# EdwardFerdian/4DFlowNet

Measured on AMD Instinct MI355X. Metric: 3D patches/sec (train step, patch=24, res×2), higher is better.
Workload: dtype f32; 1 GPU; cfg2 train_step: patch_size=24 res_increase=2 batch=8/GPU low_resblock=8 hi_resblock=4 fp32; global_batch=8, parallelism=dp1, collective=none

## Files before the change

4dflownet_amd/_lib.py:

```python
import contextlib
import ctypes
import os

from . import build as _build

_HERE = os.path.dirname(os.path.abspath(__file__))
LIB_PATH = os.path.join(_HERE, "lib4dflow_hip.so")
TEST_LIB_PATH = os.path.join(_HERE, "lib4dflow_hip_test.so")

c_fp = ctypes.c_void_p
c_i = ctypes.c_int
c_i64 = ctypes.c_int64
c_u64 = ctypes.c_uint64
c_f = ctypes.c_float
c_sz = ctypes.c_size_t

SIGNATURES = {
    "fdn_version": (c_i, []),
    "fdn_last_error": (ctypes.c_char_p, []),
    "fdn_input_features": (c_i, [c_fp] * 8 + [c_i64, c_fp]),
    "fdn_pack_conv64_weights": (c_i, [c_fp, c_fp, c_fp, c_fp]),
    "fdn_conv3d_fwd": (c_i, [c_fp] * 7 + [c_i] * 10 + [c_f, c_i, c_fp]),
    "fdn_conv3d_dgrad": (c_i, [c_fp] * 4 + [c_i] * 10 + [c_fp]),
    "fdn_conv_cout1_dgrad_folded": (c_i, [c_fp, c_fp, c_fp, c_i, c_f, c_fp, c_fp, c_fp, c_sz, c_i, c_i, c_i, c_i, c_i, c_i, c_fp]),
    "fdn_conv_cout1_dgrad_folded_mask": (c_i, [c_fp, c_fp, c_fp, c_i, c_f, c_fp, c_fp, c_fp, c_sz, c_i, c_i, c_i, c_i, c_i, c_i, c_fp]),
    "fdn_fold_halo": (c_i, [c_fp, c_fp, c_fp, c_i, c_fp, c_fp, c_i, c_f, c_fp, c_i, c_i, c_i, c_i, c_i, c_fp]),
    "fdn_conv3d_dgrad_fused": (c_i, [c_fp] * 5 + [c_i, c_f, c_fp, c_i, c_i, c_i, c_i, c_i, c_fp]),
    "fdn_conv64_mask_ok": (c_i, [c_i] * 5),
    "fdn_conv64_fwd_mask": (c_i, [c_fp] * 6 + [c_i] * 5 + [c_f, c_i, c_fp]),
    "fdn_conv64_dgrad_fused_mask": (c_i, [c_fp] * 5 + [c_i, c_f, c_fp, c_i, c_i, c_i, c_i, c_i, c_fp]),
    "fdn_conv64_dgrad_fused_multi": (c_i, [c_fp, c_fp, c_i] + [c_fp] * 4 + [c_i, c_f, c_fp, c_i, c_i, c_i, c_i, c_i, c_fp]),
    "fdn_conv3d_dgrad_fused_part": (c_i, [c_fp] * 5 + [c_i, c_f, c_fp, c_i, c_i, c_i, c_i, c_i, c_i, c_fp]),
    "fdn_fold_halo_border": (c_i, [c_fp, c_fp, c_fp, c_i, c_fp, c_fp, c_i, c_f, c_fp, c_i, c_i, c_i, c_i, c_fp]),
    "fdn_conv1x1_dgrad": (c_i, [c_fp] * 6 + [c_i64, c_fp]),
    "fdn_conv3d_wgrad_workspace_bytes": (c_sz, [c_i] * 7),
    "fdn_conv3d_wgrad_batch_workspace_bytes": (c_sz, [c_i] * 5),
    "fdn_conv3d_wgrad_batch": (c_i, [c_fp, c_fp, c_fp, c_fp, c_i, c_fp, c_sz] + [c_i] * 5 + [c_fp]),
    "fdn_conv3d_wgrad": (c_i, [c_fp] * 6 + [c_sz] + [c_i] * 10 + [c_fp]),
    "fdn_upsample_trilinear_fwd": (c_i, [c_fp, c_fp] + [c_i] * 6 + [c_fp]),
    "fdn_upsample_trilinear_bwd": (c_i, [c_fp, c_fp, c_i, c_f, c_fp] + [c_i] * 6 + [c_fp]),
    "fdn_loss_metrics": (c_i, [c_fp] * 8 + [c_i, c_i64, c_fp]),
    "fdn_loss_metrics_div": (c_i, [c_fp] * 5 + [c_f] + [c_fp] * 3 + [c_i] * 4 + [c_fp]),
    "fdn_loss_metrics_act": (c_i, [c_fp] * 5 + [c_f, c_f, c_i] + [c_fp] * 3 + [c_i] * 4 + [c_fp]),
    "fdn_loss_metrics_kind": (c_i, [c_fp] * 5 + [c_i, c_f, c_f, c_f, c_i] + [c_fp] * 3 + [c_i] * 4 + [c_fp]),
    "fdn_volume_metrics": (c_i, [c_fp, c_i, c_fp, c_fp, c_i, c_fp, c_fp] + [c_i] * 4 + [c_fp]),
    "fdn_gather_patches": (c_i, [c_fp, c_fp, c_i, c_i, c_fp]),
    "fdn_input_features_volume": (c_i, [c_fp] + [c_i] * 8 + [c_i64, c_i, c_fp, c_fp, c_fp]),
    "fdn_stitch_patches": (c_i, [c_fp, c_fp] + [c_i] * 9 + [c_i64, c_i, c_fp]),
    "fdn_stitch_patches_finish": (c_i, [c_fp, c_fp, c_fp] + [c_i] * 9 + [c_i64, c_i, c_fp]),
    "fdn_pack_patch_cores": (c_i, [c_fp, c_fp, c_i, c_i, c_i, c_fp]),
    "fdn_input_features_volume_oriented": (c_i, [c_fp] + [c_i] * 8 + [c_i64, c_i, c_i, c_i, c_fp, c_fp, c_fp]),
    "fdn_unrotate_accumulate": (c_i, [c_fp, c_fp] + [c_i] * 6 + [c_fp]),
    "fdn_input_features_volume_strided": (c_i, [c_fp] + [c_i] * 8 + [c_i64, c_i, c_i, c_i, c_i, c_fp, c_fp, c_fp]),
    "fdn_blend_patches": (c_i, [c_fp, c_fp] + [c_i] * 10 + [c_i64, c_i, c_fp]),
    "fdn_finish_volume": (c_i, [c_fp, c_fp, c_fp] + [c_i] * 4 + [c_fp]),
    "fdn_kspace_downsample_workspace_bytes": (c_sz, [c_i] * 7),
    "fdn_kspace_downsample": (c_i, [c_fp, c_fp, c_fp] + [c_i] * 7 + [c_fp, c_u64, c_u64] + [c_fp] * 5),
    "fdn_l2_sumsq": (c_i, [c_fp, c_fp, c_i64, c_fp, c_fp]),
    "fdn_adam_step": (c_i, [c_fp] * 5 + [c_i64] + [c_f] * 5 + [c_fp, c_fp, c_fp]),
    "fdn_adam_step_dev": (c_i, [c_fp] * 5 + [c_i64, c_fp] + [c_f] * 4 + [c_fp, c_fp, c_fp]),
    "fdn_adam_step_masked": (c_i, [c_fp] * 6 + [c_i64, c_f, c_fp] + [c_f] * 4 + [c_fp, c_fp, c_fp]),
    "fdn_sum_partials": (c_i, [c_fp, c_i, c_fp, c_fp]),
    "fdn_grad_accumulate": (c_i, [c_fp, c_fp, c_i64, c_i, c_fp]),
    "fdn_l2_sumsq_partials": (c_i, [c_fp, c_fp, c_i64, c_fp, c_fp]),
    "fdn_grad_sumsq_partials": (c_i, [c_fp] * 4 + [c_i64, c_f, c_fp, c_fp, c_fp]),
    "fdn_clip_scale": (c_i, [c_fp, c_i, c_f, c_fp, c_fp]),
    "fdn_adam_step_clipped": (c_i, [c_fp] * 6 + [c_i64, c_f, c_fp] + [c_f] * 4 + [c_fp, c_fp, c_f, c_fp, c_fp]),
    "fdn_adam_step_ema": (c_i, [c_fp] * 6 + [c_i64, c_f, c_fp] + [c_f] * 4 + [c_fp, c_fp, c_f, c_fp, c_f, c_i, c_fp, c_fp]),
    "fdn_pack_conv64_weights_batch": (c_i, [c_fp, c_fp, c_i, c_fp, c_fp]),
    "fdn_conv64_pack_streams": (c_i, [c_i] * 6),
    "fdn_pack_conv64_weights_batch_streams": (c_i, [c_fp, c_fp, c_i, c_fp, c_i, c_i, c_fp]),
    "fdn_pack_conv64_weights_bf16": (c_i, [c_fp, c_fp, c_fp, c_fp]),
    "fdn_pack_conv64_weights_bf16_batch": (c_i, [c_fp, c_fp, c_i, c_fp, c_fp]),
# ... 118 lines not shown
```

4dflownet_amd/csrc/elementwise.hip:

```cpp
#include "fdn_common.h"

namespace {

__device__ __forceinline__ float norm3(float a, float b, float c) {
    return sqrtf(__builtin_fmaf(c, c, __builtin_fmaf(a, a, b * b)));
}

template <typename T>
__global__ void input_features_kernel(const float* __restrict__ u, const float* __restrict__ v, const float* __restrict__ w,
                                      const float* __restrict__ mu, const float* __restrict__ mv,
                                      const float* __restrict__ mw, T* __restrict__ phase, T* __restrict__ pc, int64_t nvox) {
    for (int64_t i = (int64_t)blockIdx.x * blockDim.x + threadIdx.x; i < nvox; i += (int64_t)gridDim.x * blockDim.x) {
        const float a = u[i], b = v[i], c = w[i];
        const float ma = mu[i], mb = mv[i], mc = mw[i];
        const float speed = norm3(a, b, c);
        const float mag = norm3(ma, mb, mc);
        fdn_st1(phase + i * 3 + 0, a); fdn_st1(phase + i * 3 + 1, b); fdn_st1(phase + i * 3 + 2, c);
        fdn_st1(pc + i * 3 + 0, mag * speed); fdn_st1(pc + i * 3 + 1, mag); fdn_st1(pc + i * 3 + 2, speed);
    }
}

struct InputGeom {
    int32_t P, X, Y, Z;
    int32_t nx, ny, nz, orient;
// ... 571 lines not shown
            const float wgt = MSE ? 2.f * c0 : c0;
            const float gu = pen_psi<KIND>(du, kp, kp2) * wgt, gv = pen_psi<KIND>(dv, kp, kp2) * wgt, gw = pen_psi<KIND>(dw, kp, kp2) * wgt;
            if (out_act == FDN_ACT_TANH) tanh_grad_store(pred, g * 3, dpred + g * 3, gu, gv, gw);
            else { dpred[g * 3] = gu; dpred[g * 3 + 1] = gv; dpred[g * 3 + 2] = gw; }
        }
    }
    const float a = block_sum(sf, red);
    const float b = block_sum(snf, red);
    const float c = block_sum(srel, red);
    if (threadIdx.x == 0) {
        float* part = scratch + (size_t)gridDim.y * 8 + ((size_t)n * gridDim.x + blockIdx.x) * nparts;
        part[0] = a; part[1] = b; part[2] = c;
        if (nparts == 5) { part[3] = 0.f; part[4] = 0.f; }
    }
}

__global__ __launch_bounds__(256) __attribute__((amdgpu_waves_per_eu(7))) void loss_main_kernel(const float* __restrict__ pred, const float* __restrict__ uh,
                                                         const float* __restrict__ vh, const float* __restrict__ wh,
                                                         const float* __restrict__ mask, float* __restrict__ scratch,
                                                         float* __restrict__ dpred, int64_t V, int D, int H, int W, float div_w,
                                                         int nparts, float nf_w, int out_act, int kind, float kp) {
    __shared__ float red[4];
    if (kind == FDN_LOSS_MSE) {
        loss_body<FDN_LOSS_MSE>(pred, uh, vh, wh, mask, scratch, dpred, V, D, H, W, div_w, nparts, nf_w, out_act, 0.f, red);
        return;
    }
    int other = kind;
    asm volatile("" : "+s"(other));
    if (other == FDN_LOSS_MAE) loss_body<FDN_LOSS_MAE>(pred, uh, vh, wh, mask, scratch, dpred, V, D, H, W, div_w, nparts, nf_w, out_act, 0.f, red);
    else if (other == FDN_LOSS_HUBER) loss_body<FDN_LOSS_HUBER>(pred, uh, vh, wh, mask, scratch, dpred, V, D, H, W, div_w, nparts, nf_w, out_act, kp, red);
    else loss_body<FDN_LOSS_CHARBONNIER>(pred, uh, vh, wh, mask, scratch, dpred, V, D, H, W, div_w, nparts, nf_w, out_act, kp, red);
}

__global__ __launch_bounds__(64) void loss_finalize_kernel(const float* __restrict__ scratch, float* __restrict__ out, int N, int nblk,
                                                           int nparts, float div_w, float nf_w) {
    const int n = blockIdx.x;
    const float* part = scratch + (size_t)N * 8 + (size_t)n * nblk * nparts;
    float sf = 0.f, sn = 0.f, sr = 0.f, sdf = 0.f, sdn = 0.f;
    if (nparts == 5) {
        for (int b = threadIdx.x; b < nblk; b += 64) {
            sf += part[b * 5]; sn += part[b * 5 + 1]; sr += part[b * 5 + 2]; sdf += part[b * 5 + 3]; sdn += part[b * 5 + 4];
        }
        for (int o = 32; o > 0; o >>= 1) { sdf += __shfl_down(sdf, o, 64); sdn += __shfl_down(sdn, o, 64); }
    } else {
        for (int b = threadIdx.x; b < nblk; b += 64) { sf += part[b * 3]; sn += part[b * 3 + 1]; sr += part[b * 3 + 2]; }
    }
    for (int o = 32; o > 0; o >>= 1) { sf += __shfl_down(sf, o, 64); sn += __shfl_down(sn, o, 64); sr += __shfl_down(sr, o, 64); }
    if (threadIdx.x) return;
    const float sm = scratch[n * 8 + 0], snf = scratch[n * 8 + 1];
    const int nc = nparts == 5 ? 5 : 4;
    out[n * nc + 0] = sf / (sm + 1.f) + nf_w * (sn / (snf + 1.f));
    out[n * nc + 1] = sr / (sm + 1.f) * 100.f;
    out[n * nc + 2] = sm;
    out[n * nc + 3] = snf;
    if (nparts == 5) out[n * 5 + 4] = div_w * (sdf / (sm + 1.f) + nf_w * (sdn / (snf + 1.f)));
}

__global__ __launch_bounds__(1024) void l2_sumsq_kernel(const float* __restrict__ w, const uint8_t* __restrict__ isk,
                                                         int64_t n, float* __restrict__ out) {
    __shared__ float red[16];
    float s0 = 0.f, s1 = 0.f, s2 = 0.f, s3 = 0.f;
    int64_t i = threadIdx.x;
    for (; i + 3 * 1024 < n; i += 4 * 1024) {
        const float a0 = isk[i] ? w[i] : 0.f, a1 = isk[i + 1024] ? w[i + 1024] : 0.f;
        const float a2 = isk[i + 2048] ? w[i + 2048] : 0.f, a3 = isk[i + 3072] ? w[i + 3072] : 0.f;
        s0 += a0 * a0; s1 += a1 * a1; s2 += a2 * a2; s3 += a3 * a3;
    }
    for (; i < n; i += 1024)
// ... 267 lines not shown
    FDN_REQUIRE(hb == 1 || hb == 2, "fdn_upsample_trilinear_bwd: %d rows per block", hb);
    if (int rc = hb == 2 ? launch(std::integral_constant<int, 2>{}) : launch(std::integral_constant<int, 1>{})) return rc;
    FDN_CHECK_LAUNCH("upsample_bwd_kernel");
    return FDN_OK;
}
extern "C" int fdn_upsample_trilinear_fwd(const float* x, float* y, int N, int D, int H, int W, int C, int R, void* stream) {
    return upsample_fwd_t<float>(x, y, N, D, H, W, C, R, stream);
}
extern "C" int fdn_upsample_trilinear_bwd(const float* dy, const float* y_prev, int act, float alpha, float* dx, int N, int D,
                                          int H, int W, int C, int R, void* stream) {
    return upsample_bwd_t<float>(dy, y_prev, act, alpha, dx, N, D, H, W, C, R, stream);
}
extern "C" int fdn_upsample_trilinear_fwd_bf16(const uint16_t* x, uint16_t* y, int N, int D, int H, int W, int C, int R,
                                               void* stream) {
    return upsample_fwd_t<uint16_t>(x, y, N, D, H, W, C, R, stream);
}
extern "C" int fdn_upsample_trilinear_bwd_bf16(const uint16_t* dy, const uint16_t* y_prev, int act, float alpha, uint16_t* dx,
                                               int N, int D, int H, int W, int C, int R, void* stream) {
    return upsample_bwd_t<uint16_t>(dy, y_prev, act, alpha, dx, N, D, H, W, C, R, stream);
}

static int loss_launch(const char* who, const float* pred, const float* uh, const float* vh, const float* wh, const float* mask, float* out,
                       float* dpred, float* scratch, int N, int64_t V, int D, int H, int W, float div_w, int nparts, void* stream,
                       float nf_w = 1.f, int out_act = FDN_ACT_NONE, int kind = FDN_LOSS_MSE, float kind_param = 0.f) {
    hipStream_t s = (hipStream_t)stream;
    hipError_t e = hipMemsetAsync(scratch, 0, (size_t)N * 8 * sizeof(float), s);
    if (e != hipSuccess) { fdn_set_error("%s: memset: %s", who, hipGetErrorString(e)); return FDN_ERR_HIP; }
    const int gx = grid_for(V, FDN_LOSS_BLOCKS);
    hipLaunchKernelGGL(mask_sums_kernel, dim3(gx < 16 ? gx : 16, N), dim3(256), 0, s, mask, scratch, V);
    FDN_CHECK_LAUNCH("mask_sums_kernel");
    hipLaunchKernelGGL(loss_main_kernel, dim3(gx, N), dim3(256), 0, s, pred, uh, vh, wh, mask, scratch, dpred, V, D, H, W, div_w, nparts,
                       nf_w, out_act, kind, kind_param);
    FDN_CHECK_LAUNCH("loss_main_kernel");
    hipLaunchKernelGGL(loss_finalize_kernel, dim3(N), dim3(64), 0, s, (const float*)scratch, out, N, gx, nparts, div_w, nf_w);
    FDN_CHECK_LAUNCH("loss_finalize_kernel");
    return FDN_OK;
}

extern "C" int fdn_loss_metrics(const float* pred, const float* uh, const float* vh, const float* wh, const float* mask,
                                float* out, float* dpred, float* scratch, int N, int64_t V, void* stream) {
    FDN_REQUIRE(pred && uh && vh && wh && mask && out && scratch && N > 0 && V > 0, "fdn_loss_metrics: bad argument");
    return loss_launch("fdn_loss_metrics", pred, uh, vh, wh, mask, out, dpred, scratch, N, V, 1, 1, 1, 0.f, 3, stream);
}

extern "C" int fdn_loss_metrics_div(const float* pred, const float* uh, const float* vh, const float* wh, const float* mask,
                                    float div_weight, float* out, float* dpred, float* scratch, int N, int D, int H, int W,
                                    void* stream) {
    FDN_REQUIRE(pred && uh && vh && wh && mask && out && scratch, "fdn_loss_metrics_div: NULL operand");
    FDN_REQUIRE(N > 0 && D > 0 && H > 0 && W > 0, "fdn_loss_metrics_div: extents N=%d D=%d H=%d W=%d must be positive", N, D, H, W);
    FDN_REQUIRE((int64_t)D * H * W <= (int64_t)INT32_MAX, "fdn_loss_metrics_div: %d x %d x %d voxels per sample exceed 2^31 - 1", D, H, W);
    FDN_REQUIRE(__builtin_isfinite(div_weight) && div_weight >= 0.f, "fdn_loss_metrics_div: div_weight %g must be finite and >= 0",
                (double)div_weight);
    return loss_launch("fdn_loss_metrics_div", pred, uh, vh, wh, mask, out, dpred, scratch, N, (int64_t)D * H * W, D, H, W, div_weight, 5,
                       stream);
}

extern "C" int fdn_loss_metrics_act(const float* pred, const float* uh, const float* vh, const float* wh, const float* mask,
                                    float div_weight, float non_fluid_weight, int out_act, float* out, float* dpred, float* scratch,
                                    int N, int D, int H, int W, void* stream) {
    FDN_REQUIRE(pred && uh && vh && wh && mask && out && scratch, "fdn_loss_metrics_act: NULL operand");
    FDN_REQUIRE(N > 0 && D > 0 && H > 0 && W > 0, "fdn_loss_metrics_act: extents N=%d D=%d H=%d W=%d must be positive", N, D, H, W);
    FDN_REQUIRE((int64_t)D * H * W <= (int64_t)INT32_MAX, "fdn_loss_metrics_act: %d x %d x %d voxels per sample exceed 2^31 - 1", D, H, W);
    FDN_REQUIRE(__builtin_isfinite(div_weight) && div_weight >= 0.f, "fdn_loss_metrics_act: div_weight %g must be finite and >= 0",
                (double)div_weight);
    FDN_REQUIRE(__builtin_isfinite(non_fluid_weight) && non_fluid_weight >= 0.f,
                "fdn_loss_metrics_act: non_fluid_weight %g must be finite and >= 0", (double)non_fluid_weight);
    if (out_act != FDN_ACT_NONE && out_act != FDN_ACT_TANH) {
// ... 215 lines not shown
```

4dflownet_amd/csrc/heads_mfma.hip:

```cpp
#include "fdn_common.h"
#include <type_traits>
#include <stdlib.h>

namespace {

__device__ __forceinline__ int clampi(int v, int hi) { return min(max(v, 0), hi); }

__device__ __forceinline__ float head_tanh(float z) {
    const float a = fabsf(z);
    const float s = a * a;
    float p = __fadd_rn(__fmul_rn(-5.70498872745e-3f, s), 2.06390887954e-2f);
    p = fmaf(p, s, -5.37397155531e-2f);
    p = fmaf(p, s, 1.33314422036e-1f);
    p = fmaf(p, s, -3.33332819422e-1f);
    const float q = 0.25f * a;
    const float e = __builtin_amdgcn_exp2f(11.54156033f * (q > 4.f ? 4.f : q));
    const float t = a < 0.625f ? fmaf(p * s, a, a) : 1.f - 2.f / (e + 1.f);
    return copysignf(t, z);
}
__device__ __forceinline__ float head_act(float z, int act, float alpha) {
    if (act == FDN_ACT_TANH) return head_tanh(z);
    return fdn_act(z, act, alpha);
}

// ... 144 lines not shown
}

}

template <typename T>
int fdn_head_fwd_launch(const T* x, const float* w, const float* bias, float* y, int N, int D, int H, int W, int ldy, int y_coff,
                        int act, float alpha, hipStream_t s, int xcd_walk) {
    const int ntd = (D + H_TD - 1) / H_TD, nth = (H + H_TH - 1) / H_TH, ntw = (W + H_TW - 1) / H_TW;
    const size_t lds = (size_t)27 * H_HVP * sizeof(float);
    if (int rc = fdn_func_max_lds((const void*)head_fwd_kernel<T>, (int)lds, "head_fwd")) return rc;
    const int ntiles = N * ntd * nth * ntw;
    const int iters = 3 * ((ntiles + 3 * 512 - 1) / (3 * 512));
    const int grid = (ntiles + iters - 1) / iters;
    FDN_PLAN("fam=head_fwd op=fwd dt=%s N=%d D=%d H=%d W=%d iters=%d last=%d grid=%d tiles=%d cus=%d", sizeof(T) == 2 ? "bf16" : "f32", N, D, H, W,
             iters, ntiles - (grid - 1) * iters, grid, ntiles, fdn_plan_cus());
    hipLaunchKernelGGL(head_fwd_kernel<T>, dim3((unsigned)grid), dim3(256), lds, s, x, w, bias, y, N, D, H, W, ntd, nth, ntw, iters,
                       ldy, y_coff, act, alpha, xcd_walk);
    FDN_CHECK_LAUNCH("head_fwd_kernel");
    return FDN_OK;
}
template int fdn_head_fwd_launch<float>(const float*, const float*, const float*, float*, int, int, int, int, int, int, int, float, hipStream_t, int);
template int fdn_head_fwd_launch<uint16_t>(const uint16_t*, const float*, const float*, float*, int, int, int, int, int, int, int, float, hipStream_t, int);

namespace {

template <typename T>
__global__ __launch_bounds__(256, 2) void head_dgrad_kernel(const float* __restrict__ dz, const float* __restrict__ w,
                                                            const T* __restrict__ yprev, int act, float alpha,
                                                            T* __restrict__ out, float* __restrict__ bpart, int N, int D, int H,
                                                            int W, int ntd, int nth, int ntw, int lddz, int dz_coff,
                                                            const uint16_t* __restrict__ ymask) {
    __shared__ float zs[2][H_HV + 8];
    __shared__ float bred[4][64];
    const int tid = threadIdx.x, lane = tid & 63, wave = tid >> 6;
    const int li = lane & 31, kh = lane >> 5;
    const int tiles_per_n = ntd * nth * ntw, ntiles = N * tiles_per_n;
    const float slope = act == FDN_ACT_RELU ? 0.f : (act == FDN_ACT_LEAKY ? alpha : 1.f);

    constexpr bool VROW = sizeof(T) == 4;
    typedef __bf16 bf16x8 __attribute__((ext_vector_type(8)));
    float wa[VROW ? 2 : 1][VROW ? 14 : 1];
    bf16x8 wbh[VROW ? 1 : 2][VROW ? 1 : 2], wbl[VROW ? 1 : 2][VROW ? 1 : 2];
#pragma unroll
    for (int m = 0; m < 2; ++m) {
        const int ch = VROW ? 32 * m + li : 32 * m + 16 * ((li >> 2) & 1) + (li & 3) + 4 * (li >> 3);
        if constexpr (VROW) {
#pragma unroll
            for (int s = 0; s < 14; ++s) wa[m][s] = (2 * s + kh) < 27 ? w[(2 * s + kh) * 64 + ch] : 0.f;
        } else {
#pragma unroll
            for (int blk = 0; blk < 2; ++blk)
#pragma unroll
                for (int j = 0; j < 8; ++j) {
                    const int t = 16 * blk + 8 * kh + j;
                    const float wv = t < 27 ? w[t * 64 + ch] : 0.f;
                    const __bf16 h = (__bf16)wv;
                    wbh[m][blk][j] = h;
                    wbl[m][blk][j] = (__bf16)(wv - (float)h);
                }
        }
    }
    struct TileOrg { int n, d, h, w; };
    auto decode = [&](int tile) {
        int b = min(tile, ntiles - 1);
        TileOrg o;
        o.n = b / tiles_per_n;
// ... 13 lines not shown
            float v = 0.f;
            if ((unsigned)qd < (unsigned)D && (unsigned)qh < (unsigned)H && (unsigned)qw < (unsigned)W)
                v = dz[((size_t)o.n * D * H * W + ((size_t)qd * H + qh) * W + qw) * lddz + dz_coff];
            dst[i] = v;
        }
    };
    float bsum[2][16];
#pragma unroll
    for (int m = 0; m < 2; ++m)
#pragma unroll
        for (int r = 0; r < 16; ++r) bsum[m][r] = 0.f;

    constexpr int NST = (H_HV + 255) / 256;
    float stv[NST];
    auto stage_load = [&](const TileOrg& o) {
#pragma unroll
        for (int u = 0; u < NST; ++u) {
            const int i = tid + 256 * u;
            const int zd = i / (H_XH * H_XW);
            const int r2 = i - zd * (H_XH * H_XW);
            const int zh = r2 / H_XW;
            const int qd = o.d + zd - 1, qh = o.h + zh - 1, qw = o.w + (r2 - zh * H_XW) - 1;
            float v = 0.f;
            if (i < H_HV && (unsigned)qd < (unsigned)D && (unsigned)qh < (unsigned)H && (unsigned)qw < (unsigned)W)
                v = dz[((size_t)o.n * D * H * W + ((size_t)qd * H + qh) * W + qw) * lddz + dz_coff];
            stv[u] = v;
        }
    };
    auto stage_store = [&](float* dst) {
#pragma unroll
        for (int u = 0; u < NST; ++u)
            if (tid + 256 * u < H_HV) dst[tid + 256 * u] = stv[u];
    };
    stage(decode(blockIdx.x), zs[0]);
    int par = 0;
    for (int tile = blockIdx.x; tile < ntiles; tile += gridDim.x, par ^= 1) {
        __syncthreads();
        const bool has_next = tile + (int)gridDim.x < ntiles;
        if (has_next) stage_load(decode(tile + gridDim.x));
        const TileOrg o = decode(tile);
        const float* z = zs[par];
#pragma unroll 1
        for (int mt = wave * 2; mt < wave * 2 + 2; ++mt) {
            const int vd = mt >> 1, vh = 4 * (mt & 1) + (li >> 3), vw = li & 7;
            const int gd = o.d + vd, gh = o.h + vh, gw = o.w + vw;
            float ym[2][16];
            fdn_u32x2 ymw[VROW ? 2 : 1][VROW ? 4 : 1];
            if constexpr (VROW) {
                if (ymask) {
                    const int pw = min(o.w + 4 * kh, W - 4), ph0 = o.h + 4 * (mt & 1);
                    const size_t nv = (size_t)N * D * H * W;
                    const size_t plane = (size_t)o.n * D * H * W + (size_t)min(gd, D - 1) * H * W;
#pragma unroll
                    for (int m = 0; m < 2; ++m)
#pragma unroll
                        for (int rr = 0; rr < 4; ++rr)
                            ymw[m][rr] = *(const fdn_u32x2*)(ymask + (size_t)(2 * m + (li >> 4)) * nv + plane + (size_t)min(ph0 + rr, H - 1) * W + pw);
                } else
                if (yprev) {
                    const int pw = o.w + 4 * kh, ph0 = o.h + 4 * (mt & 1);
                    const size_t plane = (size_t)o.n * D * H * W + (size_t)min(gd, D - 1) * H * W;
#pragma unroll
                    for (int r = 0; r < 16; ++r) {
                        const size_t e = (plane + (size_t)min(ph0 + (r >> 2), H - 1) * W + min(pw + (r & 3), W - 1)) * 64 + li;
                        ym[0][r] = fdn_ld1(yprev + e);
                        ym[1][r] = fdn_ld1(yprev + e + 32);
                    }
                }
            }
            constexpr int EVP = FdnVec<T>::E;
            float yq[VROW ? 1 : 2][VROW ? 1 : 16];
            unsigned ymk[2] = {0u, 0u};
            if constexpr (!VROW) {
                if (ymask) {
                    const size_t voxp = (size_t)o.n * D * H * W + ((size_t)min(gd, D - 1) * H + min(gh, H - 1)) * W + min(gw, W - 1);
                    ymk[0] = ymask[voxp * 4 + kh];
                    ymk[1] = ymask[voxp * 4 + 2 + kh];
                } else if (yprev) {
                    const size_t voxp = (size_t)o.n * D * H * W + ((size_t)min(gd, D - 1) * H + min(gh, H - 1)) * W + min(gw, W - 1);
#pragma unroll
                    for (int m = 0; m < 2; ++m)
#pragma unroll
                        for (int r0 = 0; r0 < 16; r0 += EVP) {
                            float t[EVP];
                            FdnVec<T>::ld(yprev + voxp * 64 + 32 * m + 16 * kh + r0, t);
#pragma unroll
                            for (int q = 0; q < EVP; ++q) yq[m][r0 + q] = t[q];
                        }
                }
            }
            float nb[3][3][3];
#pragma unroll
// ... 44 lines not shown
                for (int s = 0; s < 14; ++s) {
                    const int t0 = 2 * s, t1 = 2 * s + 1;
                    const float e0 = nb[t0 / 9][(t0 / 3) % 3][t0 % 3];
                    const float e1 = t1 < 27 ? nb[t1 / 9][(t1 / 3) % 3][t1 % 3] : 0.f;
                    const float bv = kh ? e1 : e0;
                    acc[0] = __builtin_amdgcn_mfma_f32_32x32x2f32(bv, wa[0][s], acc[0], 0, 0, 0);
                    acc[1] = __builtin_amdgcn_mfma_f32_32x32x2f32(bv, wa[1][s], acc[1], 0, 0, 0);
                }
            } else {
#pragma unroll
                for (int blk = 0; blk < 2; ++blk) {
                    bf16x8 ah, al;
#pragma unroll
                    for (int j = 0; j < 8; ++j) {
                        const int t0 = 16 * blk + j, t1 = 16 * blk + 8 + j;
                        const float e0 = nb[t0 / 9][(t0 / 3) % 3][t0 % 3];
                        const float e1 = t1 < 27 ? nb[(t1 % 27) / 9][((t1 % 27) / 3) % 3][t1 % 3] : 0.f;
                        const float av = kh ? e1 : e0;
                        const __bf16 h = (__bf16)av;
                        ah[j] = h;
                        al[j] = (__bf16)(av - (float)h);
                    }
#pragma unroll
                    for (int m = 0; m < 2; ++m) {
                        acc[m] = __builtin_amdgcn_mfma_f32_32x32x16_bf16(wbh[m][blk], ah, acc[m], 0, 0, 0);
                        acc[m] = __builtin_amdgcn_mfma_f32_32x32x16_bf16(wbh[m][blk], al, acc[m], 0, 0, 0);
                        acc[m] = __builtin_amdgcn_mfma_f32_32x32x16_bf16(wbl[m][blk], ah, acc[m], 0, 0, 0);
                    }
                }
            }
            if constexpr (VROW) {
                const int pw = o.w + 4 * kh, ph0 = o.h + 4 * (mt & 1);
                const size_t plane = (size_t)o.n * D * H * W + (size_t)min(gd, D - 1) * H * W;
#pragma unroll
                for (int r = 0; r < 16; ++r) {
                    const int qh = ph0 + (r >> 2), qw = pw + (r & 3);
                    const bool in2 = gd < D && qh < H && qw < W;
                    const size_t e = (plane + (size_t)min(qh, H - 1) * W + min(qw, W - 1)) * 64 + li;
#pragma unroll
                    for (int m = 0; m < 2; ++m) {
                        float v = acc[m][r];
                        if (ymask) v *= ((ymw[m][r >> 2][(r & 3) >> 1] >> (16 * (r & 1) + (li & 15))) & 1u) ? 1.f : slope;
                        else if (yprev) v *= ym[m][r] > 0.f ? 1.f : slope;
                        if (in2) {
                            fdn_st1(out + e + 32 * m, v);
                            bsum[m][0] += v;
                        }
                    }
                }
                continue;
            }
            const bool inside = gd < D && gh < H && gw < W;
            const size_t vox = (size_t)o.n * D * H * W + ((size_t)min(gd, D - 1) * H + min(gh, H - 1)) * W + min(gw, W - 1);
#pragma unroll
            for (int m = 0; m < 2; ++m) {
                const size_t e = vox * 64 + 32 * m + 16 * kh;
                constexpr int EV = FdnVec<T>::E;
#pragma unroll
                for (int r0 = 0; r0 < 16; r0 += EV) {
                    float v[EV];
#pragma unroll
                    for (int q = 0; q < EV; ++q) v[q] = acc[m][r0 + q];
                    if (!VROW && ymask) {
#pragma unroll
                        for (int q = 0; q < EV; ++q) v[q] *= ((ymk[m] >> (r0 + q)) & 1u) ? 1.f : slope;
                    } else if (yprev) {
#pragma unroll
                        for (int q = 0; q < EV; ++q) v[q] *= yq[VROW ? 0 : m][VROW ? 0 : r0 + q] > 0.f ? 1.f : slope;
                    }
                    if (inside) {
                        FdnVec<T>::st(out + e + r0, v);
#pragma unroll
                        for (int q = 0; q < EV; ++q) bsum[m][r0 + q] += v[q];
                    }
                }
            }
        }
        if (has_next) stage_store(zs[par ^ 1]);
    }
    if (bpart && VROW) {
#pragma unroll
        for (int m = 0; m < 2; ++m) {
            float v = bsum[m][0];
            v += __shfl_xor(v, 32, 64);
            if (kh == 0) bred[wave][32 * m + li] = v;
        }
        __syncthreads();
        if (tid < 64) bpart[(size_t)blockIdx.x * 64 + tid] = (bred[0][tid] + bred[1][tid]) + (bred[2][tid] + bred[3][tid]);
    } else if (bpart) {
#pragma unroll
        for (int m = 0; m < 2; ++m)
#pragma unroll
            for (int r = 0; r < 16; ++r) {
                float v = bsum[m][r];
                v += __shfl_xor(v, 1, 64); v += __shfl_xor(v, 2, 64); v += __shfl_xor(v, 4, 64);
                v += __shfl_xor(v, 8, 64); v += __shfl_xor(v, 16, 64);
                if (li == 0) bred[wave][32 * m + 16 * kh + r] = v;
            }
        __syncthreads();
        if (tid < 64) bpart[(size_t)blockIdx.x * 64 + tid] = (bred[0][tid] + bred[1][tid]) + (bred[2][tid] + bred[3][tid]);
    }
}

}

int fdn_head_dgrad_blocks(int N, int D, int H, int W) {
    const long long ntiles = (long long)N * ((D + H_TD - 1) / H_TD) * ((H + H_TH - 1) / H_TH) * ((W + H_TW - 1) / H_TW);
    return (int)(ntiles < 1024 ? ntiles : 1024);
}

template <typename T>
// ... 330 lines not shown
```

4dflownet_amd/ops.py:

```python
import ctypes
import functools
import math
import numbers
import operator
import struct

import numpy as np
import torch

from . import _lib
from ._lib import FdnError, check

ACT_NONE, ACT_RELU, ACT_LEAKY = 0, 1, 2
ACT_TANH = 3
ALGO_AUTO, ALGO_DIRECT, ALGO_WINO_W, ALGO_WINO_H2, ALGO_WINO_BF16X3 = 0, 1, 2, 3, 4
LEAKY_ALPHA = 0.2
CONV64_PACK_FLOATS = 423 * 64 * 64
ACT_DTYPE = torch.float32
PACK_ELEMS = CONV64_PACK_FLOATS


def _ptr(dtype, t, name="tensor", allow_none=False):
    if t is None:
        if allow_none:
# ... 708 lines not shown
        raise FdnError("grad_sumsq_partials: partials needs %d floats" % ADAM_PARTIALS)
    n = g.numel()
    for name, t in (("w", w), ("is_kernel", is_kernel), ("frozen", frozen)):
        if t is not None and t.numel() != n:
            raise FdnError("grad_sumsq_partials: %s holds %d elements for %d gradients" % (name, t.numel(), n))
    if l2_scale_dev is not None and (not l2_scale_dev.is_cuda or l2_scale_dev.dtype != torch.float32 or l2_scale_dev.numel() < 1):
        raise FdnError("grad_sumsq_partials: l2_scale_dev must hold one float32 on the GPU")
    check(_lib.load().fdn_grad_sumsq_partials(_p(g, "g"), _p(w, "w"), _pu8(is_kernel, "is_kernel"), _pu8(frozen, "frozen", allow_none=True), n,
                                              float(l2_grad_scale), _p(l2_scale_dev, "l2_scale_dev", allow_none=True), _p(partials, "partials"),
                                              _stream()), "fdn_grad_sumsq_partials")
    return partials


def clip_scale(partials, clip_norm, out=None):
    c32 = ctypes.c_float(float(clip_norm)).value
    if not (c32 > 0.0 and c32 != float("inf")):
        raise FdnError("clip_scale: clip_norm must be finite and > 0 in float32, got %r" % (clip_norm,))
    clip_norm = c32
    if out is None:
        out = torch.empty((2,), device=partials.device, dtype=torch.float32)
    elif out.numel() < 2:
        raise FdnError("clip_scale: out needs 2 floats")
    check(_lib.load().fdn_clip_scale(_p(partials, "partials"), partials.numel(), clip_norm, _p(out, "out"), _stream()), "fdn_clip_scale")
    return out


def sum_partials(partials, out=None):
    if out is None:
        out = torch.empty((1,), device=partials.device, dtype=torch.float32)
    check(_lib.load().fdn_sum_partials(_p(partials), partials.numel(), _p(out), _stream()), "fdn_sum_partials")
    return out


def pack_conv64_weights_batch(w_flat, w_offsets, packs, streams=None):
    n = w_offsets.numel()
    if w_offsets.dtype != torch.int64 or not w_offsets.is_cuda or packs.numel() != n * 2 * CONV64_PACK_FLOATS:
        raise FdnError("pack_conv64_weights_batch: bad offsets / packs")
    sf, sd = (PACK_STREAM_ALL, PACK_STREAM_ALL) if streams is None else streams
    check(_lib.load().fdn_pack_conv64_weights_batch_streams(_p(w_flat), w_offsets.data_ptr(), n, _p(packs), int(sf), int(sd), _stream()),
          "fdn_pack_conv64_weights_batch_streams")
    return packs


PACK_STREAM_DIRECT, PACK_STREAM_WINO_W, PACK_STREAM_WINO_H2, PACK_STREAM_WINO_H4, PACK_STREAM_WINO_H4S = 1, 2, 4, 8, 16
PACK_STREAM_ALL = 31
ROLE_FWD, ROLE_DGRAD, ROLE_DGRAD_FUSED = 0, 1, 2


def conv64_pack_streams(N, D, H, W, algo=ALGO_AUTO, role=ROLE_FWD):
    m = _lib.load().fdn_conv64_pack_streams(int(N), int(D), int(H), int(W), int(algo), int(role))
    check(min(m, 0), "fdn_conv64_pack_streams")
    return m
```

4dflownet_amd/trainer.py:

```python
import contextlib
import ctypes
import datetime
import os
import pickle
import shutil
import time

import numpy as np
import torch

from . import ops, parallel, tfevents
from .network import Input, SR4DFlowNet

L2_LAMBDA = 5e-7
ADAM_B1, ADAM_B2, ADAM_EPS = 0.9, 0.999, 1e-7


def _clip_arguments(global_clipnorm, clipvalue):
    out = []
    for name, c in (("global_clipnorm", global_clipnorm), ("clipvalue", clipvalue)):
        if c is None:
            out.append(None)
            continue
        try:
            cf = ctypes.c_float(float(c)).value
        except (TypeError, ValueError):
            raise ValueError("%s must be None or a finite number > 0, got %r" % (name, c)) from None
        if isinstance(c, (bool, str, bytes)) or not np.isfinite(cf) or cf <= 0:
            raise ValueError("%s must be None or a finite number > 0, got %r" % (name, c))
        out.append(cf)
    if out[0] is not None and out[1] is not None:
        raise ValueError("global_clipnorm and clipvalue are both set (%r, %r): at most one kind of gradient clipping" % (global_clipnorm, clipvalue))
    return tuple(out)


def _ema_arguments(use_ema, ema_momentum, ema_overwrite_frequency, ema_validation=False):
    for name, b in (("use_ema", use_ema), ("ema_validation", ema_validation)):
        if not isinstance(b, (bool, np.bool_)):
            raise ValueError("%s must be True or False, got %r" % (name, b))
    mom = ema_momentum
    try:
        mom32 = ctypes.c_float(float(mom)).value
    except (TypeError, ValueError, OverflowError):
        raise ValueError("ema_momentum must be a real number in [0, 1) as float32, got %r" % (mom,)) from None
    if isinstance(mom, (bool, np.bool_, str, bytes)) or not 0.0 <= mom32 < 1.0:
        raise ValueError("ema_momentum must be a real number in [0, 1) as float32, got %r" % (mom,))
    k = ema_overwrite_frequency
    if k is not None and (isinstance(k, (bool, np.bool_)) or not isinstance(k, (int, np.integer)) or k < 1):
        raise ValueError("ema_overwrite_frequency must be None or an integer >= 1, got %r" % (k,))
    if ema_validation and not use_ema:
        raise ValueError("ema_validation=True validates under the averaged weights and needs use_ema=True")
    return bool(use_ema), mom32, None if k is None else int(k), bool(ema_validation)


class Mean:

    def __init__(self, name, device):
        self.name = name
        self.device = device
        self.reset_states()

    def reset_states(self):
        if getattr(self, "_total", None) is None:
            self._total = torch.zeros((), device=self.device, dtype=torch.float64)
        else:
            self._total.zero_()
        self._count = 0

    def update_state(self, values):
        if isinstance(values, torch.Tensor):
            self._total += values.sum().to(torch.float64)
            self._count += values.numel()
        else:
            self._total += float(values)
            self._count += 1

    def result(self):
        return float(self._total.item()) / self._count if self._count else 0.0

    def result_global(self):
        total, count = parallel.allreduce_sum_host([float(self._total.item()), float(self._count)])
        return total / count if count else 0.0


class _Optimizer:

    def __init__(self, model, lr):
        self.lr = float(lr)
        self.iterations = 0
        self.m = torch.zeros_like(model.flat_w)
        self.v = torch.zeros_like(model.flat_w)

    def lr_t(self):
        t = self.iterations
        return self.lr * np.sqrt(1.0 - ADAM_B2 ** t) / (1.0 - ADAM_B1 ** t)


class TrainerController:
    loss, loss_param = 'mse', None

# ... 17 lines not shown
        self._clip_partials = None
        self._clip_out = None
        self.last_grad_norm = None
        self.div_weight = div_weight
        self._checked_div_weight()
        self.accum_steps = accum_steps
        self._checked_accum_steps()
        self.accum_g_ext = None
        self._accum_k = 1
        self._accum_count = 0
        self._accum_has = False
        self.non_fluid_weight = non_fluid_weight
        self._checked_non_fluid_weight()
        self.loss = loss
        self.loss_param = loss_param
        self._checked_loss()
        self.res_increase = res_increase
        self.patch_size = patch_size
        self.QUICKSAVE_ENABLED = quicksave_enable
        self.network_name = network_name

        input_shape = (patch_size, patch_size, patch_size, 1)
        u, v, w = Input(input_shape, 'u'), Input(input_shape, 'v'), Input(input_shape, 'w')
        u_mag, v_mag, w_mag = Input(input_shape, 'u_mag'), Input(input_shape, 'v_mag'), Input(input_shape, 'w_mag')
        net = SR4DFlowNet(res_increase)
        self.model = net.build_network(u, v, w, u_mag, v_mag, w_mag, low_resblock, hi_resblock, device=device, seed=seed,
                                       dtype=dtype, conv_algo=conv_algo, output_activation=output_activation)
        self.device = self.model.device
        if trainable is not None:
            self.model.set_trainable(trainable)

        names = ['train_loss', 'val_loss', 'train_accuracy', 'val_accuracy', 'train_mse', 'val_mse', 'train_div',
                 'val_div', 'l2_reg_loss']
        self.loss_metrics = dict((n, Mean(n, self.device)) for n in names)
        self.accuracy_metric = 'val_loss'
        self.learning_rate = initial_learning_rate
        self.grad_norm_metric = Mean('grad_norm', self.device)
        self.optimizer = _Optimizer(self.model, initial_learning_rate)
        self._l2_buf = torch.zeros(1, device=self.device)
        self._l2_partials = torch.zeros(ops.ADAM_PARTIALS, device=self.device)
        self._l2_version = -1
        self.unique_model_name = network_name
        self.model_dir = None
        if bucketed_allreduce is None:
            bucketed_allreduce = os.environ.get("FDN_DP_BUCKETED", "1") not in ("0", "false", "no")
        self.bucketed_allreduce = bool(bucketed_allreduce)
        self.profile_allreduce = False
        self.allreduce_wait_events = []

    def _unpack(self, data_pairs):
        arrs = [self.model._to_dev(a) for a in data_pairs]
        u, v, w, u_mag, v_mag, w_mag, u_hr, v_hr, w_hr, venc, mask = arrs
        return (u, v, w, u_mag, v_mag, w_mag), (u_hr, v_hr, w_hr), venc, mask

    def calculate_regularizer_loss(self):
        if self._l2_version != self.model.weights_version:
            ops.l2_sumsq_partials(self.model.flat_w, self.model.is_kernel, self._l2_partials)
            self._l2_version = self.model.weights_version
        ops.sum_partials(self._l2_partials, self._l2_buf)
        return self._l2_buf[0] * L2_LAMBDA

    def _checked_div_weight(self):
        w = self.div_weight
        try:
            wf = float(w)
        except (TypeError, ValueError):
            raise ValueError("div_weight must be a finite number >= 0, got %r" % (w,)) from None
# ... 7 lines not shown
            wf = float(w)
        except (TypeError, ValueError):
            raise ValueError("non_fluid_weight must be a finite number >= 0, got %r" % (w,)) from None
        if not np.isfinite(wf) or wf < 0:
            raise ValueError("non_fluid_weight must be a finite number >= 0, got %r" % (w,))
        return wf

    def _checked_loss(self):
        kind, _, param = ops.checked_loss_kind(self.loss, self.loss_param, who="TrainerController: loss / loss_param", error=ValueError)
        return kind, (param if kind in ops.LOSS_PARAM_DEFAULTS else None)

    def _checked_accum_steps(self):
        k = self.accum_steps
        if isinstance(k, bool) or not isinstance(k, (int, np.integer)) or k < 1:
            raise ValueError("accum_steps must be an integer >= 1, got %r" % (k,))
        return int(k)

    def _checked_clip(self):
        return _clip_arguments(self.global_clipnorm, self.clipvalue)

    def _checked_ema(self):
        return _ema_arguments(self.use_ema, self.ema_momentum, self.ema_overwrite_frequency, self.ema_validation)

    def _loss_call(self, hires, predictions, mask, want_grad):
        div_weight = self._checked_div_weight()
        kind, param = self._checked_loss()
        more = {} if kind == 'mse' else {'kind': kind, 'kind_param': param}
        out, dpred = ops.loss_metrics(predictions, hires[0], hires[1], hires[2], mask, want_grad=want_grad, div_weight=div_weight,
                                      non_fluid_weight=self._checked_non_fluid_weight(), out_act=self.model.out_act, **more)
        return out, dpred, div_weight

    def calculate_and_update_metrics(self, hires, predictions, mask, metric_set, want_grad):
        out, dpred, div_weight = self._loss_call(hires, predictions, mask, want_grad)
        mse, rel_error = out[:, 0], out[:, 1]
        div = out[:, 4] if div_weight != 0 else None
        loss = mse if div is None else mse + div
        if metric_set == 'train':
            l2 = self.calculate_regularizer_loss()
            self.loss_metrics['l2_reg_loss'].update_state(l2.reshape(1))
            loss = loss + l2
        self.loss_metrics['%s_loss' % metric_set].update_state(loss)
        self.loss_metrics['%s_mse' % metric_set].update_state(mse)
        self.loss_metrics['%s_div' % metric_set].update_state(0.0 if div is None else div)
        self.loss_metrics['%s_accuracy' % metric_set].update_state(rel_error)
        return loss, dpred

    def train_step(self, data_pairs):
        if not self.model.any_trainable:
            raise ValueError("train_step: no layer of the model is trainable (layer.trainable / set_trainable), there is nothing to update")
        self._checked_clip()
        self._checked_ema()
        if self._ema_active:
            raise RuntimeError("train_step inside `with ema_weights():` -- the model holds the averaged weights, leave the context first")
        if self._accum_count == 0:
            self._accum_k = self._checked_accum_steps()
        inputs, hires, venc, mask = self._unpack(data_pairs)
        B = inputs[0].shape[0]
        m = self.model
        m.batch_slot.fill_(float(B))
        buf = self._step_buffer()
        closing = self._accum_count + 1 >= self._accum_k
        first = not self._accum_has
        contribute = None
        if self._accum_k > 1:
            def contribute(lo, hi):
                ops.grad_accumulate(buf[lo:hi], m.flat_g_ext[lo:hi], first)
        pending = on_bucket = None
        if closing and self.bucketed_allreduce and parallel.world_size() > 1:
            pending = []

            def on_bucket(lo, hi):
                if contribute is not None and B > 0:
                    contribute(lo, hi)
                pending.append(parallel.allreduce_sum_start(buf[lo:hi]))
        if B > 0:
            pred = m.forward(inputs, training=True)
            loss, dpred = self.calculate_and_update_metrics(hires, pred, mask, 'train', True)
# ... 430 lines not shown
```

include/fdn.h:

```cpp
#ifndef FDN_H
#define FDN_H
#include <stddef.h>
#include <stdint.h>
#ifdef __cplusplus
extern "C" {
#endif

#define FDN_OK 0
#define FDN_ERR_BAD_ARG (-1)
#define FDN_ERR_UNSUPPORTED (-2)
#define FDN_ERR_HIP (-3)
#define FDN_ERR_WORKSPACE (-4)

#define FDN_ACT_NONE 0
#define FDN_ACT_RELU 1
#define FDN_ACT_LEAKY 2
#define FDN_ACT_TANH 3

#define FDN_ALGO_AUTO 0
#define FDN_ALGO_DIRECT 1
#define FDN_ALGO_WINO_W 2
#define FDN_ALGO_WINO_H2 3
#define FDN_ALGO_WINO_BF16X3 4
#define FDN_ALGO_LAST FDN_ALGO_WINO_BF16X3
// ... 65 lines not shown
size_t fdn_conv3d_wgrad_workspace_bytes(int N, int D, int H, int W, int Cin, int Cout, int K);

size_t fdn_conv3d_wgrad_batch_workspace_bytes(int n_layers, int N, int D, int H, int W);
int fdn_conv3d_wgrad_batch(const float* const* x, const float* const* dz, float* const* dw, float* const* dbias, int n_layers,
                           void* workspace, size_t workspace_bytes, int N, int D, int H, int W, int algo, void* stream);
int fdn_conv3d_wgrad(const float* x, const float* x2, const float* dz, float* dw, float* dbias,
                     void* workspace, size_t workspace_bytes, int N, int D, int H, int W, int Cin, int Cout,
                     int K, int lddz, int dz_coff, int algo, void* stream);

int fdn_upsample_trilinear_fwd(const float* x, float* y, int N, int D, int H, int W, int C, int R, void* stream);
int fdn_upsample_trilinear_bwd(const float* dy, const float* y_prev, int act, float alpha, float* dx, int N,
                               int D, int H, int W, int C, int R, void* stream);

#define FDN_LOSS_BLOCKS 256
#define FDN_LOSS_SCRATCH_FLOATS(N) ((N) * (8 + 3 * FDN_LOSS_BLOCKS))
int fdn_loss_metrics(const float* pred, const float* uh, const float* vh, const float* wh, const float* mask,
                     float* out, float* dpred, float* scratch, int N, int64_t V, void* stream);

#define FDN_LOSS_DIV_SCRATCH_FLOATS(N) ((N) * (8 + 5 * FDN_LOSS_BLOCKS))
int fdn_loss_metrics_div(const float* pred, const float* uh, const float* vh, const float* wh, const float* mask,
                         float div_weight, float* out, float* dpred, float* scratch, int N, int D, int H, int W, void* stream);

int fdn_loss_metrics_act(const float* pred, const float* uh, const float* vh, const float* wh, const float* mask, float div_weight,
                         float non_fluid_weight, int out_act, float* out, float* dpred, float* scratch, int N, int D, int H, int W,
                         void* stream);

#define FDN_LOSS_MSE 0
#define FDN_LOSS_MAE 1
#define FDN_LOSS_HUBER 2
#define FDN_LOSS_CHARBONNIER 3
int fdn_loss_metrics_kind(const float* pred, const float* uh, const float* vh, const float* wh, const float* mask, int kind,
                          float kind_param, float div_weight, float non_fluid_weight, int out_act, float* out, float* dpred,
                          float* scratch, int N, int D, int H, int W, void* stream);

#define FDN_VOLUME_METRICS_COLUMNS 26
#define FDN_VOLUME_METRICS_SCRATCH_DOUBLES(F) ((F) * FDN_VOLUME_METRICS_COLUMNS * FDN_LOSS_BLOCKS)
int fdn_volume_metrics(const void* pred, int pred_is_f64, const float* truth, const float* mask, int mask_frames,
                       double* out, double* scratch, int F, int X, int Y, int Z, void* stream);

int fdn_gather_patches(const void* desc, float* out, int B, int S, void* stream);

int fdn_input_features_volume(const float* frames, int F, int X, int Y, int Z, int P, int nx, int ny, int nz, int64_t g0,
                              int count, float* phase, float* pc, void* stream);
int fdn_stitch_patches(const float* pred, float* vol, int F, int Xo, int Yo, int Zo, int S, int side, int nx, int ny, int nz,
                       int64_t g0, int count, void* stream);
int fdn_stitch_patches_finish(const float* pred, double* vol, const double* frame_scale, int F, int Xo, int Yo, int Zo,
                              int S, int side, int nx, int ny, int nz, int64_t g0, int count, void* stream);
int fdn_pack_patch_cores(const float* pred, float* cores, int S, int side, int count, void* stream);

int fdn_input_features_volume_oriented(const float* frames, int F, int X, int Y, int Z, int P, int nx, int ny, int nz, int64_t g0,
                                       int count, int plane, int k, float* phase, float* pc, void* stream);
int fdn_unrotate_accumulate(const float* pred, float* acc, int count, int S, int plane, int k, int first, int divisor, void* stream);

int fdn_input_features_volume_strided(const float* frames, int F, int X, int Y, int Z, int P, int nx, int ny, int nz, int64_t g0,
                                      int count, int stride, int plane, int k, float* phase, float* pc, void* stream);
int fdn_blend_patches(const float* pred, float* acc, int F, int Xo, int Yo, int Zo, int S, int side, int stride_hr, int nx, int ny, int nz,
                      int64_t g0, int count, void* stream);
int fdn_finish_volume(const float* acc, double* vol, const double* frame_scale, int F, int Xo, int Yo, int Zo, void* stream);

size_t fdn_kspace_downsample_workspace_bytes(int nvol, int X, int Y, int Z, int cx, int cy, int cz);
int fdn_kspace_downsample(const float* vel, const float* mag, const float* params, int nvol, int X, int Y, int Z, int cx, int cy, int cz,
                          const float* noise, uint64_t seed, uint64_t stream_id, float* out_vel, float* out_mag, float* sigma_out,
                          void* workspace, void* stream);

int fdn_l2_sumsq(const float* w, const uint8_t* is_kernel, int64_t n, float* out, void* stream);

// ... 87 lines not shown
```

Before: 333.9 patches/s.

## Fuse per-step metric accumulation into one kernel and prefetch head masks into LDS

Replaces the chain of small torch ops that computed loss, mse, div and accuracy means with one single-block kernel launch. That kernel writes the per-sample loss and adds into shared float64 totals, and the Mean objects become views into those totals. Separately, the MFMA head kernel now prefetches the next tile's y-mask into a double-buffered LDS array alongside the existing stage load, instead of issuing scattered global loads inside the inner loop. This reduces launch overhead and global-load latency, but adds LDS use and a serialized shuffle reduction.

```diff
diff --git a/4dflownet_amd/_lib.py b/4dflownet_amd/_lib.py
--- a/4dflownet_amd/_lib.py
+++ b/4dflownet_amd/_lib.py
@@ -39,6 +39,7 @@
     "fdn_conv3d_wgrad": (c_i, [c_fp] * 6 + [c_sz] + [c_i] * 10 + [c_fp]),
     "fdn_upsample_trilinear_fwd": (c_i, [c_fp, c_fp] + [c_i] * 6 + [c_fp]),
     "fdn_upsample_trilinear_bwd": (c_i, [c_fp, c_fp, c_i, c_f, c_fp] + [c_i] * 6 + [c_fp]),
+    "fdn_step_metrics": (c_i, [c_fp, c_i, c_i, c_i, c_fp, c_fp, c_fp, c_fp]),
     "fdn_loss_metrics": (c_i, [c_fp] * 8 + [c_i, c_i64, c_fp]),
     "fdn_loss_metrics_div": (c_i, [c_fp] * 5 + [c_f] + [c_fp] * 3 + [c_i] * 4 + [c_fp]),
     "fdn_loss_metrics_act": (c_i, [c_fp] * 5 + [c_f, c_f, c_i] + [c_fp] * 3 + [c_i] * 4 + [c_fp]),
diff --git a/4dflownet_amd/csrc/elementwise.hip b/4dflownet_amd/csrc/elementwise.hip
--- a/4dflownet_amd/csrc/elementwise.hip
+++ b/4dflownet_amd/csrc/elementwise.hip
@@ -627,8 +627,35 @@
     else loss_body<FDN_LOSS_CHARBONNIER>(pred, uh, vh, wh, mask, scratch, dpred, V, D, H, W, div_w, nparts, nf_w, out_act, kp, red);
 }
 
+struct LossStep { const float* l2; float* loss; double* totals; int ncols, has_div; };
+__device__ __forceinline__ void loss_step_stage(const float* __restrict__ out, int N, const LossStep& step) {
+    const float l2v = step.l2 ? step.l2[0] : 0.f;
+    double sl = 0.0, sm = 0.0, sd = 0.0, sa = 0.0;
+    for (int b0 = 0; b0 < N; b0 += 64) {
+        const int b = b0 + (int)threadIdx.x;
+        float v = 0.f, o0 = 0.f, o1 = 0.f, o4 = 0.f;
+        if (b < N) {
+            const float* o = out + (size_t)b * step.ncols;
+            o0 = o[0]; o1 = o[1];
+            v = o0;
+            if (step.has_div) { o4 = o[4]; v = v + o4; }
+            if (step.l2) v = v + l2v;
+            step.loss[b] = v;
+        }
+        const int cnt = min(64, N - b0);
+        for (int j = 0; j < cnt; ++j) {
+            sl += (double)__shfl(v, j, 64); sm += (double)__shfl(o0, j, 64);
+            sd += (double)__shfl(o4, j, 64); sa += (double)__shfl(o1, j, 64);
+        }
+    }
+    if (threadIdx.x) return;
+    step.totals[0] += sl; step.totals[1] += sm; step.totals[3] += sa;
+    if (step.has_div) step.totals[2] += sd;
+    if (step.l2) step.totals[4] += (double)l2v;
+}
 __global__ __launch_bounds__(64) void loss_finalize_kernel(const float* __restrict__ scratch, float* __restrict__ out, int N, int nblk,
-                                                           int nparts, float div_w, float nf_w) {
+                                                           int nparts, float div_w, float nf_w, LossStep step) {
+    if (step.loss) { loss_step_stage(out, N, step); return; }
     const int n = blockIdx.x;
     const float* part = scratch + (size_t)N * 8 + (size_t)n * nblk * nparts;
     float sf = 0.f, sn = 0.f, sr = 0.f, sdf = 0.f, sdn = 0.f;
@@ -962,7 +989,20 @@
     hipLaunchKernelGGL(loss_main_kernel, dim3(gx, N), dim3(256), 0, s, pred, uh, vh, wh, mask, scratch, dpred, V, D, H, W, div_w, nparts,
                        nf_w, out_act, kind, kind_param);
     FDN_CHECK_LAUNCH("loss_main_kernel");
-    hipLaunchKernelGGL(loss_finalize_kernel, dim3(N), dim3(64), 0, s, (const float*)scratch, out, N, gx, nparts, div_w, nf_w);
+    hipLaunchKernelGGL(loss_finalize_kernel, dim3(N), dim3(64), 0, s, (const float*)scratch, out, N, gx, nparts, div_w, nf_w, LossStep{});
+    FDN_CHECK_LAUNCH("loss_finalize_kernel");
+    return FDN_OK;
+}
+
+extern "C" int fdn_step_metrics(const float* out, int ncols, int N, int has_div, const float* l2_dev, float* loss, double* totals,
+                                void* stream) {
+    FDN_REQUIRE(out && loss && totals, "fdn_step_metrics: NULL operand");
+    FDN_REQUIRE(N > 0 && (ncols == 4 || ncols == 5), "fdn_step_metrics: N=%d samples of %d columns (4 or 5)", N, ncols);
+    FDN_REQUIRE(has_div == 0 || (has_div == 1 && ncols == 5), "fdn_step_metrics: has_div=%d needs the 5-column out of fdn_loss_metrics_div (ncols=%d)",
+                has_div, ncols);
+    const LossStep step{l2_dev, loss, totals, ncols, has_div};
+    hipLaunchKernelGGL(loss_finalize_kernel, dim3(1), dim3(64), 0, (hipStream_t)stream, (const float*)nullptr, const_cast<float*>(out), N, 0, 0,
+                       0.f, 0.f, step);
     FDN_CHECK_LAUNCH("loss_finalize_kernel");
     return FDN_OK;
 }
diff --git a/4dflownet_amd/csrc/heads_mfma.hip b/4dflownet_amd/csrc/heads_mfma.hip
--- a/4dflownet_amd/csrc/heads_mfma.hip
+++ b/4dflownet_amd/csrc/heads_mfma.hip
@@ -200,6 +200,7 @@
                                                             const uint16_t* __restrict__ ymask) {
     __shared__ float zs[2][H_HV + 8];
     __shared__ float bred[4][64];
+    __shared__ fdn_u32x2 ms[2][sizeof(T) == 4 ? 256 : 1];
     const int tid = threadIdx.x, lane = tid & 63, wave = tid >> 6;
     const int li = lane & 31, kh = lane >> 5;
     const int tiles_per_n = ntd * nth * ntw, ntiles = N * tiles_per_n;
@@ -279,12 +280,21 @@
         for (int u = 0; u < NST; ++u)
             if (tid + 256 * u < H_HV) dst[tid + 256 * u] = stv[u];
     };
+    const bool use_ms = VROW && ymask != nullptr;
+    auto mask_load = [&](const TileOrg& o) {
+        const int p = tid >> 6, sd = (tid >> 4) & 3, sh = (tid >> 1) & 7;
+        const size_t vox = (size_t)o.n * D * H * W + ((size_t)min(o.d + sd, D - 1) * H + min(o.h + sh, H - 1)) * W + min(o.w + 4 * (tid & 1), W - 4);
+        return *(const fdn_u32x2*)(ymask + (size_t)p * ((size_t)N * D * H * W) + vox);
+    };
+    fdn_u32x2 msv = {0u, 0u};
     stage(decode(blockIdx.x), zs[0]);
+    if (use_ms) ms[0][VROW ? tid : 0] = mask_load(decode(blockIdx.x));
     int par = 0;
     for (int tile = blockIdx.x; tile < ntiles; tile += gridDim.x, par ^= 1) {
         __syncthreads();
         const bool has_next = tile + (int)gridDim.x < ntiles;
         if (has_next) stage_load(decode(tile + gridDim.x));
+        if (has_next && use_ms) msv = mask_load(decode(tile + gridDim.x));
         const TileOrg o = decode(tile);
         const float* z = zs[par];
 #pragma unroll 1
@@ -294,17 +304,7 @@
             float ym[2][16];
             fdn_u32x2 ymw[VROW ? 2 : 1][VROW ? 4 : 1];
             if constexpr (VROW) {
-                if (ymask) {
-                    const int pw = min(o.w + 4 * kh, W - 4), ph0 = o.h + 4 * (mt & 1);
-                    const size_t nv = (size_t)N * D * H * W;
-                    const size_t plane = (size_t)o.n * D * H * W + (size_t)min(gd, D - 1) * H * W;
-#pragma unroll
-                    for (int m = 0; m < 2; ++m)
-#pragma unroll
-                        for (int rr = 0; rr < 4; ++rr)
-                            ymw[m][rr] = *(const fdn_u32x2*)(ymask + (size_t)(2 * m + (li >> 4)) * nv + plane + (size_t)min(ph0 + rr, H - 1) * W + pw);
-                } else
-                if (yprev) {
+                if (!ymask && yprev) {
                     const int pw = o.w + 4 * kh, ph0 = o.h + 4 * (mt & 1);
                     const size_t plane = (size_t)o.n * D * H * W + (size_t)min(gd, D - 1) * H * W;
 #pragma unroll
@@ -415,6 +415,13 @@
             if constexpr (VROW) {
                 const int pw = o.w + 4 * kh, ph0 = o.h + 4 * (mt & 1);
                 const size_t plane = (size_t)o.n * D * H * W + (size_t)min(gd, D - 1) * H * W;
+                if (ymask) {
+#pragma unroll
+                    for (int m = 0; m < 2; ++m)
+#pragma unroll
+                        for (int rr = 0; rr < 4; ++rr)
+                            ymw[m][rr] = ms[par][(((2 * m + (li >> 4)) * 4 + vd) * 8 + 4 * (mt & 1) + rr) * 2 + kh];
+                }
 #pragma unroll
                 for (int r = 0; r < 16; ++r) {
                     const int qh = ph0 + (r >> 2), qw = pw + (r & 3);
@@ -460,6 +467,7 @@
             }
         }
         if (has_next) stage_store(zs[par ^ 1]);
+        if (has_next && use_ms) ms[par ^ 1][VROW ? tid : 0] = msv;
     }
     if (bpart && VROW) {
 #pragma unroll
diff --git a/4dflownet_amd/ops.py b/4dflownet_amd/ops.py
--- a/4dflownet_amd/ops.py
+++ b/4dflownet_amd/ops.py
@@ -764,6 +764,21 @@
     return out
 
 
+def step_metrics(out, totals, has_div=False, l2=None, loss=None):
+    N, ncols = out.shape
+    if out.dtype != torch.float32 or not out.is_contiguous():
+        raise FdnError("step_metrics: out must be the contiguous fp32 (N, 4 or 5) of loss_metrics")
+    if totals.dtype != torch.float64 or totals.numel() != 5 or not totals.is_contiguous() or totals.device != out.device:
+        raise FdnError("step_metrics: totals must be 5 contiguous float64 on out's device")
+    if l2 is not None and (l2.dtype != torch.float32 or l2.numel() != 1 or l2.device != out.device):
+        raise FdnError("step_metrics: l2 must be one fp32 value on out's device")
+    if loss is None:
+        loss = torch.empty((N,), device=out.device, dtype=torch.float32)
+    check(_lib.load().fdn_step_metrics(_p(out, "out"), ncols, N, int(bool(has_div)), _p(l2, "l2", allow_none=True), _p(loss, "loss"),
+                                       _ptr(torch.float64, totals, "totals"), _stream()), "fdn_step_metrics")
+    return loss
+
+
 def pack_conv64_weights_batch(w_flat, w_offsets, packs, streams=None):
     n = w_offsets.numel()
     if w_offsets.dtype != torch.int64 or not w_offsets.is_cuda or packs.numel() != n * 2 * CONV64_PACK_FLOATS:
diff --git a/4dflownet_amd/trainer.py b/4dflownet_amd/trainer.py
--- a/4dflownet_amd/trainer.py
+++ b/4dflownet_amd/trainer.py
@@ -55,9 +55,10 @@
 
 class Mean:
 
-    def __init__(self, name, device):
+    def __init__(self, name, device, total=None):
         self.name = name
         self.device = device
+        self._total = total
         self.reset_states()
 
     def reset_states(self):
@@ -66,6 +67,9 @@
         else:
             self._total.zero_()
         self._count = 0
+
+    def count_state(self, n):
+        self._count += n
 
     def update_state(self, values):
         if isinstance(values, torch.Tensor):
@@ -149,7 +153,9 @@
 
         names = ['train_loss', 'val_loss', 'train_accuracy', 'val_accuracy', 'train_mse', 'val_mse', 'train_div',
                  'val_div', 'l2_reg_loss']
-        self.loss_metrics = dict((n, Mean(n, self.device)) for n in names)
+        self._metric_totals = torch.zeros((2, 5), device=self.device, dtype=torch.float64)
+        slot = lambda n: (0, 4) if n == 'l2_reg_loss' else (('train', 'val').index(n.split('_')[0]), ('loss', 'mse', 'div', 'accuracy').index(n.split('_')[1]))
+        self.loss_metrics = dict((n, Mean(n, self.device, total=self._metric_totals[slot(n)])) for n in names)
         self.accuracy_metric = 'val_loss'
         self.learning_rate = initial_learning_rate
         self.grad_norm_metric = Mean('grad_norm', self.device)
@@ -223,17 +229,17 @@
 
     def calculate_and_update_metrics(self, hires, predictions, mask, metric_set, want_grad):
         out, dpred, div_weight = self._loss_call(hires, predictions, mask, want_grad)
-        mse, rel_error = out[:, 0], out[:, 1]
-        div = out[:, 4] if div_weight != 0 else None
-        loss = mse if div is None else mse + div
-        if metric_set == 'train':
-            l2 = self.calculate_regularizer_loss()
-            self.loss_metrics['l2_reg_loss'].update_state(l2.reshape(1))
-            loss = loss + l2
-        self.loss_metrics['%s_loss' % metric_set].update_state(loss)
-        self.loss_metrics['%s_mse' % metric_set].update_state(mse)
-        self.loss_metrics['%s_div' % metric_set].update_state(0.0 if div is None else div)
-        self.loss_metrics['%s_accuracy' % metric_set].update_state(rel_error)
+        train = metric_set == 'train'
+        has_div = div_weight != 0
+        l2 = self.calculate_regularizer_loss() if train else None
+        loss = ops.step_metrics(out, self._metric_totals[0 if train else 1], has_div=has_div, l2=l2)
+        B = out.shape[0]
+        if train:
+            self.loss_metrics['l2_reg_loss'].count_state(1)
+        self.loss_metrics['%s_loss' % metric_set].count_state(B)
+        self.loss_metrics['%s_mse' % metric_set].count_state(B)
+        self.loss_metrics['%s_div' % metric_set].count_state(B if has_div else 1)
+        self.loss_metrics['%s_accuracy' % metric_set].count_state(B)
         return loss, dpred
 
     def train_step(self, data_pairs):
diff --git a/include/fdn.h b/include/fdn.h
--- a/include/fdn.h
+++ b/include/fdn.h
@@ -121,6 +121,8 @@
 int fdn_loss_metrics_kind(const float* pred, const float* uh, const float* vh, const float* wh, const float* mask, int kind,
                           float kind_param, float div_weight, float non_fluid_weight, int out_act, float* out, float* dpred,
                           float* scratch, int N, int D, int H, int W, void* stream);
+int fdn_step_metrics(const float* out, int ncols, int N, int has_div, const float* l2_dev , float* loss, double* totals,
+                     void* stream);
 
 #define FDN_VOLUME_METRICS_COLUMNS 26
 #define FDN_VOLUME_METRICS_SCRATCH_DOUBLES(F) ((F) * FDN_VOLUME_METRICS_COLUMNS * FDN_LOSS_BLOCKS)
```

After: 335.0 patches/s (median of 6 runs). About the same (+0.3%).
